# ethz-asl/laser_slam

Measured on AMD Instinct MI355X. Metric: scans_per_sec, higher is better.
Workload: dtype f32

## Files before the change

### devtools/ne_phases.py

```python
import ctypes as C, sys, os
ROOT = os.path.dirname(os.path.dirname(os.path.abspath(__file__)))
sys.path.insert(0, ROOT)
os.environ["LSGPU_SO"] = os.path.join(ROOT, "devtools", "liblsgpu_stats.so")
import numpy as np, torch
from laser_slam_amd import synth, icp
from laser_slam_amd._lib import IcpConfig, lib
n_az = int(sys.argv[1]) if len(sys.argv) > 1 else 16384
ref, rd, Tt, Ti = synth.scan_pair(n_az)
cfg = IcpConfig(); lib().lsgpu_icp_config_yaml(C.byref(cfg)); cfg.min_diff_rot, cfg.min_diff_trans = 1e-5, 1e-4
h = icp.IcpHandle(cfg)
dref, dn = h.filter_reference(torch.from_numpy(ref).cuda(), 10, 1.0, 0)
dref, dn = dref.clone(), dn.clone()
drd = torch.from_numpy(rd).cuda()
L = lib()
L.lsgpu_dev_ne_phases.argtypes = [C.c_void_p, C.POINTER(C.c_ulonglong)]
buf = (C.c_ulonglong * 24)()
h.set_reference(dref, dn); T, st = h.align(drd, Ti)
L.lsgpu_dev_ne_phases(h._h, buf); a0 = np.array(list(buf), np.float64)
h.set_reference(dref, dn); T, st = h.align(drd, Ti)
L.lsgpu_dev_ne_phases(h._h, buf); a1 = np.array(list(buf), np.float64)
d = a1 - a0
n, blocks = d[0], d[4]
print("launches %d, blocks per launch %.0f, iterations %d" % (n, blocks / n, st.iterations))
print("per block (shader cycles): prologue %.0f | main loop %.0f | wave+block reduce, hand-off %.0f" % (d[1] / blocks, d[2] / blocks, d[3] / blocks))
print("wall (us, 100 MHz clock): first start -> first loop start %.2f | first start -> last loop end %.2f | last loop end -> kernel end %.2f (update lane %.2f)"
      % (d[9] / n / 100, d[7] / n / 100, d[8] / n / 100, d[11] / n / 100))
print("tail (us): last loop end -> last block knows it is last %.2f | partials + state + set-aside loads, first sums %.2f | set-aside ranking + sums %.2f | final sums, publish %.2f" % tuple(d[16:20] / n / 100))
print("update lane (shader cycles per launch): unpack + LLT %.0f | delta, T update %.0f | trace record %.0f | checker %.0f" % tuple(d[12:16] / n))
print("distances set aside per iteration (stats build):", [t["searching"] for t in h.trace()])
```

### laser_slam_amd/csrc/lsgpu_host_math.h

```cpp
#pragma once
#include <cmath>
#include <cstring>

#if defined(__HIPCC__)
#define LSGPU_HD __host__ __device__ inline
#else
#define LSGPU_HD inline
#endif

namespace lsgpu {
namespace hostmath {

LSGPU_HD float at(const float* m, int r, int c) { return m[c * 4 + r]; }
LSGPU_HD void set(float* m, int r, int c, float v) { m[c * 4 + r] = v; }

LSGPU_HD void identity4(float* m) {
  for (int i = 0; i < 16; ++i) m[i] = (i % 5 == 0) ? 1.f : 0.f;
}

LSGPU_HD void mul4(const float* a, const float* b, float* out) {
  float t[16];
  for (int c = 0; c < 4; ++c)
    for (int r = 0; r < 4; ++r) {
      float s = at(a, r, 0) * at(b, 0, c);
// ... 158 lines not shown
    q[0] = 0.5f * t;
    t = 0.5f / t;
    q[1] = (at(T, 2, 1) - at(T, 1, 2)) * t;
    q[2] = (at(T, 0, 2) - at(T, 2, 0)) * t;
    q[3] = (at(T, 1, 0) - at(T, 0, 1)) * t;
  } else {
    int i = 0;
    if (at(T, 1, 1) > at(T, 0, 0)) i = 1;
    if (at(T, 2, 2) > at(T, i, i)) i = 2;
    const int j = (i + 1) % 3, k = (j + 1) % 3;
    t = sqrtf(at(T, i, i) - at(T, j, j) - at(T, k, k) + 1.0f);
    q[1 + i] = 0.5f * t;
    t = 0.5f / t;
    q[0] = (at(T, k, j) - at(T, j, k)) * t;
    q[1 + j] = (at(T, j, i) + at(T, i, j)) * t;
    q[1 + k] = (at(T, k, i) + at(T, i, k)) * t;
  }
}

LSGPU_HD float angular_distance(const float a[4], const float b[4]) {
  const float bw = b[0], bx = -b[1], by = -b[2], bz = -b[3];
  const float w = a[0] * bw - a[1] * bx - a[2] * by - a[3] * bz;
  const float x = a[0] * bx + a[1] * bw + a[2] * bz - a[3] * by;
  const float y = a[0] * by + a[2] * bw + a[3] * bx - a[1] * bz;
  const float z = a[0] * bz + a[3] * bw + a[1] * by - a[2] * bx;
  return 2.0f * atan2_f32(sqrtf(x * x + y * y + z * z), fabsf(w));
}

struct CheckerState {
  int counter;
  int n_hist;
};

LSGPU_HD void checker_push(CheckerState* s, float* hist, const float* T) {
  float* e = hist + 8 * s->n_hist;
  quat_from_rotation(T, e);
  e[4] = at(T, 0, 3); e[5] = at(T, 1, 3); e[6] = at(T, 2, 3);
  e[7] = s->n_hist > 0 ? fabsf(angular_distance(e, e - 8)) : 0.f;
  s->n_hist++;
}

LSGPU_HD bool checker_check(CheckerState* s, float* hist, int max_iter, int smooth, float lim_rot,
                            float lim_trans, const float* T, bool* iterate, bool* by_diff, float* out2 = nullptr) {
  if (out2) { out2[0] = 0.f; out2[1] = 0.f; }
  if (++s->counter >= max_iter) { *iterate = false; return true; }
  checker_push(s, hist, T);
  float rot = 0.f, trans = 0.f;
  const int n = s->n_hist;
  if (n > smooth) {
    for (int i = n - 1; i >= n - smooth; --i) {
      const float* a = hist + 8 * i;
      const float* b = hist + 8 * (i - 1);
      rot += a[7];
      const float dx = a[4] - b[4], dy = a[5] - b[5], dz = a[6] - b[6];
      trans += fabsf(sqrtf(dx * dx + dy * dy + dz * dz));
    }
    rot /= (float)smooth;
    trans /= (float)smooth;
    if (out2) { out2[0] = rot; out2[1] = trans; }
    if (rot < lim_rot && trans < lim_trans) { *iterate = false; *by_diff = true; }
  }
  return !(rot != rot || trans != trans);
}

}
}
```

### laser_slam_amd/csrc/lsgpu_icp.hip

```cpp
#include <cstring>
#include <cmath>
#include <cstdio>
#include <cstdlib>
#include <string>
#include <vector>
#include <chrono>
#include <functional>
#include <system_error>
#include <thread>
#include <utility>

#include <dlfcn.h>

#include <hip/hip_runtime.h>
#include <rccl/rccl.h>

#include "../../include/lsgpu_icp.h"
#include "lsgpu_grid.hip.h"
#include "lsgpu_tuning.h"
#include "lsgpu_policy.h"
#include "lsgpu_knn.hip.h"
#include "lsgpu_knn_k.hip.h"
#include "lsgpu_snf.hip.h"
#include "lsgpu_cone.hip.h"
// ... 2686 lines not shown
    pc.kmatch = kmatch; pc.chain = chain;
    pc.robust_mad = robust && ca.rb.mad; pc.robust_scale_iters = robust ? h->robust.nb_iteration_for_scale : 0;
    if (h->cone_build_in_align) { h->cone_ok = cone_wanted(h); h->cone_decided = false; }
    if (h->index_rest > 0 && (h->nr > 2 * h->index_rest_nr || 2 * h->nr < h->index_rest_nr)) h->index_rest = 0;
    const bool index_rests = h->index_rest > 0 && h->cone_ok;
    if (index_rests) { --h->index_rest; if (h->cone_build_in_align) { h->cone_build_in_align = false; h->cone_ok = false; } }
    h->pol.begin_align(h->cone_ok && !index_rests, h->cone_decided, h->cone_dense, h->cone_occupancy);
    h->pay_voxel_timed = h->pay_index_timed = false;
    if (!h->ev_pay[0]) for (auto& e : h->ev_pay) HIPC(hipEventCreate(&e));
    if (pc.lookahead && !pc.comm && !h->ev_state) HIPC(hipEventCreateWithFlags(&h->ev_state, hipEventDisableTiming));
    return LSGPU_OK;
  }

  int enqueue_iteration(const policy::Iteration& itn) {
    int r = LSGPU_OK;
    if (kmatch || chain) {
      const int np = (int)(kk * nq);
      r = run_knn_k(h, kk, Tdummy, h->state.p, itn.seed, timed);
      if (r) return r;
      ev_of_launch.push_back(h->knn_events_used ? h->knn_events_used - 1 : 0);
      r = run_select(h, h->kd2.p, np, k, false , h->state.p, true, false, 3,
                     chain ? h->cfg.trim_ratio : 0.f, chain && (ca.has_median || itn.mad));
      if (r) return r;
      if (itn.mad) { r = run_mad(h, h->kd2.p, np, h->state.p); if (r) return r; }
      ChainArgs ca_it = ca;
      ca_it.rb_recompute = itn.mad ? 1 : 0;
      lsgpu_icp::KnnEv* evk = (timed && h->knn_events_used) ? &h->knn_events[h->knn_events_used - 1] : nullptr;
      if (evk) HIPC(hipEventRecord(evk->d, h->stream));
      hipLaunchKernelGGL(ne_loop_k, dim3(nb), dim3(256), 0, h->stream, h->rdq.p, np,
                         h->state.p, h->kmatch.p, h->kd2.p, (p2p && !(robust && ca.rb.plane) && !angle) ? (const float4*)nullptr : h->nrm.p, h->hist.p, h->sel.p + 2,
                         h->counters.p + 32, h->ne_tickets.p, h->ne_partials.p, h->ne_gpartials.p, h->ne_out.p,
                         h->chk_hist.p, h->trace_dev.p, max_it, 0, (split_update && !robust && !angle) ? 0 : 1,
                         h->sel_aux.p, (uint32_t*)nullptr, 0, (uint32_t*)nullptr,
                         0, (uint32_t*)nullptr, (uint2*)nullptr, (double*)nullptr, 0, 0, ca_it);
      if (split_update && !robust && !angle)
        hipLaunchKernelGGL(update, dim3(1), dim3(64), 0, h->stream, h->state.p, h->ne_out.p,
                           h->chk_hist.p, h->trace_dev.p, max_it, 0, h->sel_aux.p);
      if (evk) HIPC(hipEventRecord(evk->e, h->stream));
      return hipGetLastError() == hipSuccess ? LSGPU_OK : LSGPU_HIP_ERROR;
    }
    if (itn.knn) {
      r = run_knn(h, Tdummy, h->state.p, itn, timed, itn.seed && itn.capped ? k : 0xFFFFFFFFu);
      if (r) return r;
      ev_of_launch.push_back(h->knn_events_used ? h->knn_events_used - 1 : 0);
    }
    if (itn.committed && h->comm) {
      RcclApi* api = rccl_api();
      comm_mark(h, true);
      if (api->GroupStart) RCCLC(api->GroupStart());
      RCCLC(api->AllReduce(h->sel_aux.p, h->sel_aux.p, kSelFailFlag, ncclUint32, ncclSum, h->comm, h->stream));
      RCCLC(api->AllReduce(h->hist.p + kHistBins, h->hist.p + kHistBins, kHistBins, ncclUint32, ncclSum, h->comm, h->stream));
      RCCLC(api->AllReduce(h->sel_win.p, h->sel_win.p, (size_t)kSelWinRows * 512, ncclUint32, ncclSum, h->comm, h->stream));
      if (api->GroupEnd) RCCLC(api->GroupEnd());
      comm_mark(h, false);
    }
    if (!itn.committed) {
      r = run_select(h, h->d2.p, (int)nq, k, false ,
                     h->state.p, true, itn.predicted, itn.full_select ? 3 : 2);
      if (r) return r;
    }
    lsgpu_icp::KnnEv* ev = (timed && itn.knn && h->knn_events_used) ? &h->knn_events[h->knn_events_used - 1] : nullptr;
    if (ev) HIPC(hipEventRecord(ev->d, h->stream));
    hipLaunchKernelGGL(ne_loop, dim3(nb), dim3(256), 0, h->stream, h->rdq.p, (int)nq,
                       h->state.p, h->prev.p, h->d2.p, p2p ? (const float4*)nullptr : h->nrm.p, h->hist.p, h->sel.p + 2,
                       h->counters.p + 32, h->ne_tickets.p, h->ne_partials.p, h->ne_gpartials.p, h->ne_out.p,
                       h->chk_hist.p, h->trace_dev.p, max_it, itn.capped ? 1 : 0, (h->comm || split_update) ? 0 : 1,
                       h->sel_aux.p, (h->comm || !tuning().fused_select) ? h->sel_win.p : nullptr, itn.committed ? 1 : 0, h->spread_cnt.p,
                       (itn.predicted && itn.knn) ? 1 : 0, h->sel_aux.p + kSelFailFlag + 2, h->amb_key.p, h->amb_val.p, tuning().sel_amb_cap,
                       (!itn.full_select && !itn.committed) ? 1 : 0, ChainArgs{});
    if (h->comm || split_update) {
      if (h->comm) comm_mark(h, true);
      if (h->comm && rccl_api()->AllReduce(h->ne_out.p, h->ne_out.p, kNe, ncclDouble, ncclSum, h->comm, h->stream) != ncclSuccess) {
        h->err = "RCCL all-reduce of the normal equations failed";
        return LSGPU_HIP_ERROR;
      }
      if (h->comm) comm_mark(h, false);
      hipLaunchKernelGGL(update, dim3(1), dim3(64), 0, h->stream, h->state.p, h->ne_out.p,
                         h->chk_hist.p, h->trace_dev.p, max_it, itn.capped ? 1 : 0, h->sel_aux.p);
    }
    if (ev) HIPC(hipEventRecord(ev->e, h->stream));
    return hipGetLastError() == hipSuccess ? LSGPU_OK : LSGPU_HIP_ERROR;
  }

  int fetch_state(int* enqueued_ahead) {
    *enqueued_ahead = 0;
    HIPC(hipMemcpyAsync(hst, h->state.p, sizeof(IcpState), hipMemcpyDeviceToHost, h->stream));
    policy::Iteration ahead_it;
    if (h->pol.lookahead_iteration(h->pol_cfg, &ahead_it)) {
      HIPC(hipEventRecord(h->ev_state, h->stream));
      const int r = enqueue_iteration(ahead_it);
      if (r) return r;
      *enqueued_ahead = 1;
      HIPC(hipEventSynchronize(h->ev_state));
      return LSGPU_OK;
    }
    return wait_stream(h);
  }

  int feed() {
    policy::Config& pc = h->pol_cfg;
    policy::State& pol = h->pol;
    int rc = enqueue_iteration(pol.plan(pc, true, pc.seed_cap && pc.cap_enabled, true, true, false));
// ... 264 lines not shown
```

### laser_slam_amd/csrc/lsgpu_solve.hip.h

```cpp
#pragma once
#include "lsgpu_common.hip.h"
#include "lsgpu_host_math.h"
#include "lsgpu_robust.h"
#include "lsgpu_normal_angle.h"
#include "../../include/lsgpu_icp.h"

namespace lsgpu {

struct SelState {
  uint32_t prefix;
  uint32_t k;
};

__device__ void find_bin(const uint32_t* __restrict__ hist, int nbins, uint32_t k, uint32_t* bin,
                         uint32_t* krem, uint32_t* sh ) {
  const int t = threadIdx.x, lane = t & 63, w = t >> 6;
  const int per = nbins / 256;
  uint32_t c[16];
  uint32_t loc = 0;
#pragma unroll
  for (int i = 0; i < 16; ++i) { c[i] = i < per ? hist[t * per + i] : 0u; loc += c[i]; }
  uint32_t incl = loc;
#pragma unroll
  for (int o = 1; o < 64; o <<= 1) {
// ... 342 lines not shown
      acc[28] += wd * ((double)res * (double)res);
      continue;
    }
    int k = 0;
#pragma unroll
    for (int a = 0; a < 6; ++a) {
#pragma unroll
      for (int c = a; c < 6; ++c) acc[k++] += (double)J[a] * (double)J[c];
    }
#pragma unroll
    for (int a = 0; a < 6; ++a) acc[21 + a] -= (double)J[a] * (double)res;
    acc[27] += 1.0;
    acc[28] += (double)res * (double)res;
  }
#pragma unroll
  for (int k = 0; k < kNe; ++k) acc[k] = ne_slot_unused<MIN>(k) ? 0.0 : wave_sum(acc[k]);
  const int w = threadIdx.x >> 6;
  if ((threadIdx.x & 63) == 0) {
#pragma unroll
    for (int k = 0; k < kNe; ++k) red[w][k] = acc[k];
  }
  __syncthreads();
  if (threadIdx.x < kNe)
    partials[(size_t)blockIdx.x * 32 + threadIdx.x] =
        ((red[0][threadIdx.x] + red[1][threadIdx.x]) + red[2][threadIdx.x]) + red[3][threadIdx.x];
}

constexpr float kCapFactor = 1.1f;

#ifdef LSGPU_KNN_STATS
__device__ unsigned long long g_ne_dbg[24] = {0, 0, 0, 0, 0, ~0ull, 0, 0, 0, 0, ~0ull, 0, 0, 0, 0, 0, 0, 0, 0, 0, 0, 0, 0, 0};
__device__ unsigned long long g_ne_tail[4];
#endif
template <int MIN, bool RB = false>
__device__ inline void icp_update_lane(IcpState* st, const double* ne_out, float* chk_hist,
                                       lsgpu_iter_trace* trace, int trace_cap, int capped_launch,
                                       uint32_t* sel_aux, int sel_failed = -1 ,
                                       const RobustIter* rb = nullptr) {
  if (st->done) return;
  if (sel_failed < 0) {
    sel_failed = (sel_aux && sel_aux[kSelFailFlag]) ? 1 : 0;
    if (sel_failed) sel_aux[kSelFailFlag] = 0u;
  }
  if (sel_failed) {
    st->sel_mode = 0;
    st->sel_fails += 1;
    st->status = kStatusSelFailed;
    st->done = 1;
    return;
  }
  const float limit = (float)ne_out[29];
  const unsigned long long nstrag = (unsigned long long)ne_out[30];
  if (capped_launch && st->cap2 < INFINITY && !(limit <= st->cap2)) {
    st->status = kStatusCapFailed;
    st->done = 1;
    return;
  }
#ifdef LSGPU_KNN_STATS
  const long long u0 = clock64();
#endif
  st->stragglers += nstrag;
  long long used = (long long)ne_out[27];
  if constexpr (RB) {
    used = rb->used;
    if (rb->mad && !(rb->scale > 0.f && rb->scale < INFINITY)) { st->status = LSGPU_NO_CONVERGENCE; st->err_code = 5; st->done = 1; return; }
    if (rb->bad > 0.0) { st->status = LSGPU_NO_CONVERGENCE; st->err_code = 6; st->done = 1; return; }
  }
  if (used <= 0) { st->status = LSGPU_NO_CONVERGENCE; st->err_code = 1; st->done = 1; return; }
  double A[36], b[6];
  float x[6], dT[16], Tn[16];
  double xd[6];
// ... 36 lines not shown
  }
  if constexpr (RB) rb->state->scale = rb->scale;
#ifdef LSGPU_KNN_STATS
  const long long u3 = clock64();
#endif
  {
    const uint32_t lb = __float_as_uint(limit), b1 = lb >> 20, b2 = (lb >> 9) & 0x7FFu;
    if (st->sel_wide) {
      const float prev = st->prev_limit;
      const bool armed = limit > 1e-30f && limit < 1e30f && prev < 1e30f && limit >= kSelArmLo * prev && limit <= kSelArmHi * prev && st->sel_fails < 2;
      const float move = armed ? fabsf(limit - prev) / prev : 1.f;
      const float f_lo = fmaxf(kSelWideLo, 1.f - 4.f * move - 0.01f), f_hi = fminf(2.f * kSelWideLo, 1.f + 4.f * move + 0.01f);
      const uint32_t lo_s = __float_as_uint(limit * f_lo) >> kSelSliceShift, hi_s = (__float_as_uint(limit * f_hi) >> kSelSliceShift) + 1u;
      st->sel_lo = lo_s << kSelSliceShift;
      st->sel_span = (hi_s - lo_s < (uint32_t)kSelSlices ? hi_s - lo_s : (uint32_t)kSelSlices) << kSelSliceShift;
      st->sel_shift = kSelSliceShift;
      st->sel_streak = armed ? st->sel_streak + 1 : 0;
      st->sel_mode = armed ? 1 : 0;
    } else {
      const uint32_t moved = b2 > st->sel_bin2 ? b2 - st->sel_bin2 : st->sel_bin2 - b2;
      st->sel_streak = (b1 == st->sel_bin1 && moved <= (uint32_t)kSelStreakBins) ? st->sel_streak + 1 : 0;
      st->sel_mode = (b1 == st->sel_bin1) ? 1 : 0;
      st->sel_lo = b1 << 20; st->sel_span = 1u << 20; st->sel_shift = 9;
    }
    st->sel_bin1 = b1;
    st->sel_bin2 = b2;
  }
  st->prev_limit = limit;
  st->cap2 = st->cap_enabled ? limit * kCapFactor : INFINITY;
  st->iter = it + 1;
  hostmath::CheckerState cs{st->counter, st->n_hist};
  bool iterate = true, by_diff = false;
  float chk2[2];
  const bool ok = hostmath::checker_check(&cs, chk_hist, st->max_iter, st->smooth, st->lim_rot,
                                          st->lim_trans, Tn, &iterate, &by_diff, chk2);
  st->chk_rot_prev = st->chk_rot; st->chk_trans_prev = st->chk_trans;
  st->chk_rot = chk2[0]; st->chk_trans = chk2[1];
  st->counter = cs.counter; st->n_hist = cs.n_hist;
#ifdef LSGPU_KNN_STATS
  {
    const long long u4 = clock64();
    g_ne_dbg[12] += (unsigned long long)(u1 - u0); g_ne_dbg[13] += (unsigned long long)(u2 - u1);
    g_ne_dbg[14] += (unsigned long long)(u3 - u2); g_ne_dbg[15] += (unsigned long long)(u4 - u3);
  }
#endif
  if (!ok) { st->status = LSGPU_NO_CONVERGENCE; st->err_code = 3; st->done = 1; return; }
  if (!iterate) { st->converged = by_diff ? 1 : 0; st->done = 1; }
}

template <int MIN>
__global__ __launch_bounds__(64) void k_icp_update(IcpState* __restrict__ st,
                                                   const double* __restrict__ ne_out,
                                                   float* __restrict__ chk_hist,
                                                   lsgpu_iter_trace* __restrict__ trace, int trace_cap,
                                                   int capped_launch, uint32_t* __restrict__ sel_aux) {
  if (threadIdx.x == 0) icp_update_lane<MIN>(st, ne_out, chk_hist, trace, trace_cap, capped_launch, sel_aux);
}


#ifndef LSGPU_NE_UNROLL
#define LSGPU_NE_UNROLL 8
#endif
constexpr int kNeUnroll = LSGPU_NE_UNROLL;
template <int MIN, int KP = 1, bool CHAIN = false, bool RB = false>
__global__ __launch_bounds__(256) void k_normal_eq_loop(const float4* __restrict__ rdq, int nq,
                                                        IcpState* __restrict__ ist,
                                                        const float4* __restrict__ match,
                                                        const float* __restrict__ d2,
                                                        const float4* __restrict__ nrm,
                                                        uint32_t* __restrict__ hist,
                                                        const SelState* __restrict__ st,
                                                        uint32_t* __restrict__ strag_count,
                                                        uint32_t* __restrict__ ticket,
                                                        double* __restrict__ partials,
                                                        double* __restrict__ gpartials,
                                                        double* __restrict__ out ,
                                                        float* __restrict__ chk_hist,
                                                        lsgpu_iter_trace* __restrict__ trace, int trace_cap,
                                                        int capped_launch, int fuse_update,
                                                        uint32_t* __restrict__ sel_aux,
                                                        uint32_t* __restrict__ hist3w ,
                                                        int committed,
                                                        uint32_t* __restrict__ spread_cnt ,
                                                        int predicted ,
                                                        uint32_t* __restrict__ amb_cnt, uint2* __restrict__ amb_key ,
                                                        double* __restrict__ amb_val ,
                                                        int amb_cap ,
                                                        int two_pass ,
                                                        ChainArgs chain ) {
  __shared__ uint32_t sc[260];
  __shared__ double fin[32];
  __shared__ double red[8][33];
  __shared__ int is_last;
  if (ist->done) return;
  const bool wide = ist->sel_wide && amb_cnt;
  const bool fused = wide && (committed || (predicted && ist->sel_mode));
  const bool plain2 = wide && !fused && two_pass;
  const bool resolve = fused || plain2;
  uint32_t s_slice = 0xFFFFFFFFu;
  uint32_t f_krem2 = 0u, f_cnt2 = 0u;
#ifdef LSGPU_KNN_STATS
  const long long c0 = clock64();
  if (threadIdx.x == 0) atomicMin(&g_ne_dbg[5], (unsigned long long)wall_clock64());
#endif
  Mat34 T;
#pragma unroll
  for (int i = 0; i < 12; ++i) T.m[i] = ist->T_rows[i];
  float limit;
  bool sel_ok = true;
  if (fused) {
    __shared__ uint32_t wsum[4], fres[4];
    const int t = threadIdx.x, lane = t & 63, w = t >> 6;
    const uint4* h4 = reinterpret_cast<const uint4*>(hist + kHistBins) + t * (kSelSlices / 256 / 4);
    static_assert(kSelSlices == 256 * 16, "16 slices per thread");
    uint4 c4[4];
#pragma unroll
    for (int i = 0; i < 4; ++i) c4[i] = h4[i];
    uint32_t bel = t < kSelBelowSlots ? sel_aux[t * kSelBelowStride] : 0u;
    const uint32_t k = st[-2].k;
    uint32_t c[16];
#pragma unroll
    for (int i = 0; i < 4; ++i) { c[4 * i] = c4[i].x; c[4 * i + 1] = c4[i].y; c[4 * i + 2] = c4[i].z; c[4 * i + 3] = c4[i].w; }
    uint32_t loc = 0u;
#pragma unroll
    for (int i = 0; i < 16; ++i) loc += c[i];
    uint32_t incl = loc;
#pragma unroll
// ... 74 lines not shown
    if constexpr (RB) { if (!chain.has_trim) limit = INFINITY; }
    if constexpr (CHAIN) {
      if (chain.has_median) limit = fminf(limit, chain.med_factor * select_limit(chain.hist_med + 2 * kHistBins, chain.sel_med + 2, sc));
      limit = fminf(limit, chain.max2);
    }
    if (wide) {
      const uint32_t lb = __float_as_uint(limit), sl = lb >> kSelSliceShift;
      const uint32_t i0 = (sl << (kSelSliceShift - 9)) & (uint32_t)(kHistBins - 1);
      uint32_t cnt = 0u;
      for (uint32_t i = 0; i < (1u << (kSelSliceShift - 9)); ++i) cnt += hist[kHistBins + i0 + i];
      if (cnt <= (uint32_t)amb_cap) { s_slice = sl; f_cnt2 = cnt; }
    }
  }
#ifdef LSGPU_KNN_STATS
  const long long c1 = clock64();
  if (threadIdx.x == 0) atomicMin(&g_ne_dbg[10], (unsigned long long)wall_clock64());
#endif
  float rb_scale = 1.f, rb_med = 0.f;
  double rb_cnt = 0.0, rb_bad = 0.0;
  if constexpr (RB) {
    if (chain.rb.mad) {
      rb_med = chain.rb_state->median;
      if (chain.rb_recompute) rb_scale = sqrtf(select_limit(chain.rb_hist + 2 * kHistBins, chain.rb_sel + 2, sc));
      else rb_scale = chain.rb_state->scale;
    }
  }
  const bool rb_normals = MIN != kPointToPoint || (RB && chain.rb.plane);
  const float* na_rn = nullptr;
  if constexpr (CHAIN) na_rn = chain.na_rn;
  double na_rej = 0.0;
  double acc[kNe];
#pragma unroll
  for (int k = 0; k < kNe; ++k) acc[k] = 0.0;
  const int stride = gridDim.x * 256;
  for (int j0 = blockIdx.x * 256 + threadIdx.x; j0 < (sel_ok ? nq : 0); j0 += kNeUnroll * stride) {
    float dd[kNeUnroll]; float4 qq[kNeUnroll], rr[kNeUnroll], nn[kNeUnroll]; bool use[kNeUnroll], amb[kNeUnroll];
#pragma unroll
    for (int u = 0; u < kNeUnroll; ++u) {
      const int j = j0 + u * stride;
      use[u] = j < nq;
      dd[u] = use[u] ? d2[j] : INFINITY;
      {
        const uint32_t sl = __float_as_uint(dd[u]) >> kSelSliceShift;
        const bool in_s = sl == s_slice;
        bool inl = resolve ? sl <= s_slice : dd[u] <= limit;
        if constexpr (CHAIN) inl = inl && chain.lo2 <= dd[u];
        amb[u] = use[u] && inl && in_s;
        use[u] = use[u] && inl;
      }
      qq[u] = use[u] ? match[j] : make_float4(0.f, 0.f, 0.f, __int_as_float(-1));
      if constexpr (KP > 1) rr[u] = use[u] ? rdq[j / KP] : make_float4(0.f, 0.f, 0.f, 0.f);
      else rr[u] = use[u] ? rdq[j] : make_float4(0.f, 0.f, 0.f, 0.f);
      use[u] = use[u] && __float_as_int(qq[u].w) >= 0;
    }
#pragma unroll
    for (int u = 0; u < kNeUnroll; ++u) {
      if constexpr (MIN != kPointToPoint) nn[u] = use[u] ? nrm[__float_as_int(qq[u].w)] : make_float4(0.f, 0.f, 0.f, 0.f);
      else if constexpr (RB) nn[u] = (use[u] && (rb_normals || na_rn)) ? nrm[__float_as_int(qq[u].w)] : make_float4(0.f, 0.f, 0.f, 0.f);
      else if constexpr (CHAIN) nn[u] = (use[u] && na_rn) ? nrm[__float_as_int(qq[u].w)] : make_float4(0.f, 0.f, 0.f, 0.f);
    }
#pragma unroll
    for (int u = 0; u < kNeUnroll; ++u) {
    if (!use[u]) continue;
    const float4 q = qq[u];
    const float4 r = rr[u];
    if constexpr (CHAIN) {
      if (na_rn) {
        const float* rn = na_rn + 3 * (size_t)__float_as_uint(r.w);
        if (!normal_angle::keep(T.m, rn[0], rn[1], rn[2], nn[u].x, nn[u].y, nn[u].z, chain.na_eps)) { na_rej += 1.0; continue; }
      }
    }
    const float3 p = xform(T, r.x, r.y, r.z);
    if constexpr (MIN == kPointToPoint) {
      double v[16];
// ... 58 lines not shown
                           __ATOMIC_RELAXED, __HIP_MEMORY_SCOPE_AGENT);
      }
      continue;
    }
    if constexpr (RB) {
      const float wf = robust::weight(chain.rb.fct, chain.rb.plane ? res * res : dd[u], rb_scale, chain.rb.k, chain.rb.approx2);
      if (!(fabsf(wf) < INFINITY)) { rb_bad += 1.0; continue; }
      if (!(wf > 0.f)) continue;
      rb_cnt += 1.0;
      const double wd = (double)wf;
      int k = 0;
#pragma unroll
      for (int a = 0; a < 6; ++a) {
#pragma unroll
        for (int c = a; c < 6; ++c) acc[k++] += wd * ((double)J[a] * (double)J[c]);
      }
#pragma unroll
      for (int a = 0; a < 6; ++a) acc[21 + a] -= wd * ((double)J[a] * (double)res);
      acc[27] += wd;
      acc[28] += wd * ((double)res * (double)res);
      continue;
    }
    int k = 0;
#pragma unroll
    for (int a = 0; a < 6; ++a) {
#pragma unroll
      for (int c = a; c < 6; ++c) acc[k++] += (double)J[a] * (double)J[c];
    }
#pragma unroll
    for (int a = 0; a < 6; ++a) acc[21 + a] -= (double)J[a] * (double)res;
    acc[27] += 1.0;
    acc[28] += (double)res * (double)res;
    }
  }
#ifdef LSGPU_KNN_STATS
  asm volatile("s_waitcnt vmcnt(0)" ::: "memory");
  const long long c2 = clock64();
  if (threadIdx.x == 0) atomicMax(&g_ne_dbg[6], (unsigned long long)wall_clock64());
#endif
#pragma unroll
  for (int k = 0; k < kNe; ++k) acc[k] = ne_slot_unused<MIN>(k) ? 0.0 : wave_sum(acc[k]);
  const int w = threadIdx.x >> 6;
  if constexpr (RB) { rb_cnt = wave_sum(rb_cnt); rb_bad = wave_sum(rb_bad); }
  if constexpr (CHAIN) { if (na_rn) na_rej = wave_sum(na_rej); }
  if ((threadIdx.x & 63) == 0) {
#pragma unroll
    for (int k = 0; k < kNe; ++k) red[w][k] = acc[k];
    if constexpr (RB) { red[w][29] = rb_cnt; red[w][30] = rb_bad; }
    if constexpr (CHAIN) red[w][31] = na_rej;
  }
  __syncthreads();
  if (threadIdx.x < (RB ? kNe + 2 : kNe) || (CHAIN && threadIdx.x == 31))
    __hip_atomic_store(&partials[(size_t)blockIdx.x * 32 + threadIdx.x],
                       ((red[0][threadIdx.x] + red[1][threadIdx.x]) + red[2][threadIdx.x]) + red[3][threadIdx.x],
                       __ATOMIC_RELAXED, __HIP_MEMORY_SCOPE_AGENT);
#if (defined(__gfx950__) || defined(__gfx942__)) && !defined(LSGPU_NE_FENCED)
  asm volatile("s_waitcnt vmcnt(0)" ::: "memory");
#else
  __builtin_amdgcn_fence(__ATOMIC_RELEASE, "agent");
  asm volatile("s_waitcnt vmcnt(0)" ::: "memory");
#endif
  __syncthreads();
  if (threadIdx.x == 0) {
    const uint32_t t = __hip_atomic_fetch_add(ticket, 1u, __ATOMIC_RELAXED, __HIP_MEMORY_SCOPE_AGENT);
    is_last = (t == gridDim.x - 1);
#ifdef LSGPU_KNN_STATS
    const long long c3 = clock64();
    atomicAdd(&g_ne_dbg[1], (unsigned long long)(c1 - c0)); atomicAdd(&g_ne_dbg[2], (unsigned long long)(c2 - c1));
    atomicAdd(&g_ne_dbg[3], (unsigned long long)(c3 - c2)); atomicAdd(&g_ne_dbg[4], 1ull);
#endif
  }
  __syncthreads();
  if (!is_last) return;
#ifdef LSGPU_KNN_STATS
  if (threadIdx.x == 0) g_ne_tail[0] = (unsigned long long)wall_clock64();
#endif
#if !((defined(__gfx950__) || defined(__gfx942__)) && !defined(LSGPU_NE_FENCED))
  __builtin_amdgcn_fence(__ATOMIC_ACQUIRE, "agent");
#endif
  __shared__ IcpState st_sh;
  __shared__ uint32_t fail_sh, cnt_sh[2];
  constexpr int kStWords = (int)(sizeof(IcpState) / sizeof(uint32_t));
  uint32_t* sw = reinterpret_cast<uint32_t*>(&st_sh);
  uint32_t* gw = reinterpret_cast<uint32_t*>(ist);
  uint32_t st_word[(kStWords + 255) / 256];
  if (fuse_update) {
#pragma unroll
    for (int i = 0; i < (kStWords + 255) / 256; ++i)
      st_word[i] = (int)threadIdx.x + 256 * i < kStWords ? gw[threadIdx.x + 256 * i] : 0u;
  }
  const bool s_on = sel_ok && s_slice != 0xFFFFFFFFu;
  __shared__ __attribute__((aligned(16))) uint32_t akj[kSelAmbCap];
  __shared__ __attribute__((aligned(16))) uint32_t akb[kSelAmbCap];
  __shared__ uint32_t aord[kSelAmbCap];
  __shared__ uint32_t alim_sh, am_sh;
  __shared__ double red2[8][33];
  constexpr int kAmbLds = 64;
  __shared__ double aval[kAmbLds * 32];
  uint32_t an = 0u;
  unsigned long long akey = 0ull;
  double av[kAmbLds * 32 / 256];
  if (s_on) {
    an = __hip_atomic_load(amb_cnt, __ATOMIC_RELAXED, __HIP_MEMORY_SCOPE_AGENT);
    const uint32_t kmax = f_cnt2 ? f_cnt2 - 1u : 0u, vmax = kmax * 32u + 31u;
    akey = __hip_atomic_load(reinterpret_cast<unsigned long long*>(&amb_key[threadIdx.x < kmax ? threadIdx.x : kmax]), __ATOMIC_RELAXED, __HIP_MEMORY_SCOPE_AGENT);
#pragma unroll
    for (int u = 0; u < kAmbLds * 32 / 256; ++u) {
      const uint32_t i = threadIdx.x + 256u * (uint32_t)u;
      av[u] = __hip_atomic_load(&amb_val[i < vmax ? i : vmax], __ATOMIC_RELAXED, __HIP_MEMORY_SCOPE_AGENT);
    }
  }
  uint32_t fail_word = 0u, ns_word = 0u, nw_word = 0u;
  if (threadIdx.x == 255) {
    if (sel_aux) fail_word = sel_aux[kSelFailFlag];
    ns_word = __hip_atomic_load(strag_count, __ATOMIC_RELAXED, __HIP_MEMORY_SCOPE_AGENT);
    nw_word = __hip_atomic_load(strag_count + 2, __ATOMIC_RELAXED, __HIP_MEMORY_SCOPE_AGENT);
  }
  {
    const int col = threadIdx.x & 31, slice = threadIdx.x >> 5;
    const uint32_t per = (gridDim.x + 7u) / 8u;
    const uint32_t r0 = (uint32_t)slice * per, r1 = r0 + per < gridDim.x ? r0 + per : gridDim.x;
    double t = 0.0;
    uint32_t r = r0;
    for (; r + 16 <= r1; r += 16) {
      double v[16];
#pragma unroll
      for (int u = 0; u < 16; ++u)
        v[u] = __hip_atomic_load(&partials[(size_t)(r + u) * 32 + col], __ATOMIC_RELAXED, __HIP_MEMORY_SCOPE_AGENT);
#pragma unroll
      for (int u = 0; u < 16; ++u) t += v[u];
    }
    for (; r < r1; ++r)
      t += __hip_atomic_load(&partials[(size_t)r * 32 + col], __ATOMIC_RELAXED, __HIP_MEMORY_SCOPE_AGENT);
    red[slice][col] = t;
  }
  if (fuse_update) {
#pragma unroll
    for (int i = 0; i < (kStWords + 255) / 256; ++i)
      if ((int)threadIdx.x + 256 * i < kStWords) sw[threadIdx.x + 256 * i] = st_word[i];
  }
  if (s_on) {
#pragma unroll
    for (int u = 0; u < kAmbLds * 32 / 256; ++u) aval[threadIdx.x + 256 * u] = av[u];
    const uint32_t n_in = an < (uint32_t)kSelAmbCap ? an : (uint32_t)kSelAmbCap;
    akj[threadIdx.x] = threadIdx.x < n_in ? (uint32_t)akey : 0xFFFFFFFFu;
    akb[threadIdx.x] = threadIdx.x < n_in ? (uint32_t)(akey >> 32) : 0xFFFFFFFFu;
    if (threadIdx.x == 0) { alim_sh = resolve ? 0xFFFFFFFFu : __float_as_uint(limit); am_sh = 0u; }
  }
  __syncthreads();
#ifdef LSGPU_KNN_STATS
  if (threadIdx.x == 0) g_ne_tail[1] = (unsigned long long)wall_clock64();
#endif
  bool amb_ok = true;
  if (s_on) {
    if (resolve) amb_ok = an == f_cnt2;
    const uint32_t n = amb_ok ? (an < (uint32_t)kSelAmbCap ? an : (uint32_t)kSelAmbCap) : 0u;
    const uint32_t mb = akb[threadIdx.x], mj = akj[threadIdx.x];
    if (resolve) {
      if (threadIdx.x < n) {
        uint32_t cl = 0u, cle = 0u;
        for (uint32_t e0 = 0; e0 < n; e0 += 8u) {
          const uint4 b0 = *reinterpret_cast<const uint4*>(&akb[e0]), b1 = *reinterpret_cast<const uint4*>(&akb[e0 + 4u]);
          const uint32_t eb[8] = {b0.x, b0.y, b0.z, b0.w, b1.x, b1.y, b1.z, b1.w};
#pragma unroll
          for (int q = 0; q < 8; ++q) { cl += eb[q] < mb ? 1u : 0u; cle += eb[q] <= mb ? 1u : 0u; }
        }
        if (cl <= f_krem2 && f_krem2 < cle) alim_sh = mb;
      }
      __syncthreads();
    }
    const uint32_t lim_bits = alim_sh;
    amb_ok = amb_ok && lim_bits != 0xFFFFFFFFu;
    limit = __uint_as_float(lim_bits);
// ... 66 lines not shown
#ifdef LSGPU_KNN_STATS
    const double nw_dbg = s_on ? (double)an : nw;
    out[31] = nw_dbg; fin[31] = nw_dbg;
#else
    out[31] = nw; fin[31] = nw;
#endif
    __hip_atomic_store(strag_count, 0u, __ATOMIC_RELAXED, __HIP_MEMORY_SCOPE_AGENT);
    __hip_atomic_store(strag_count + 2, 0u, __ATOMIC_RELAXED, __HIP_MEMORY_SCOPE_AGENT);
    __hip_atomic_store(ticket, 0u, __ATOMIC_RELAXED, __HIP_MEMORY_SCOPE_AGENT);
    if (spread_cnt) {
      const uint32_t n = __hip_atomic_load(spread_cnt + 1, __ATOMIC_RELAXED, __HIP_MEMORY_SCOPE_AGENT);
      const uint32_t nc = n < (uint32_t)kFrontMax ? n : (uint32_t)kFrontMax;
      __hip_atomic_store(spread_cnt, nc, __ATOMIC_RELAXED, __HIP_MEMORY_SCOPE_AGENT);
      if (fuse_update) st_sh.n_spread = nc; else ist->n_spread = nc;
    }
  }
#ifdef LSGPU_KNN_STATS
  unsigned long long w_pre = 0;
  if (threadIdx.x == 0) w_pre = (unsigned long long)wall_clock64();
#endif
  __syncthreads();
  if (threadIdx.x == 0) {
    if constexpr (CHAIN) {
      if (na_rn && chain.na_trace && !st_sh.done && st_sh.iter < trace_cap) {
        lsgpu_normal_angle_trace& nt = chain.na_trace[st_sh.iter];
        nt.rejected = (long long)red[2][32]; nt.eps = chain.na_eps; nt.reserved = 0;
      }
    }
    if constexpr (RB) {
      RobustIter ri;
      ri.used = (long long)red[0][32]; ri.bad = red[1][32]; ri.scale = rb_scale; ri.median = rb_med;
      ri.recomputed = (chain.rb.mad && chain.rb_recompute) ? 1 : 0; ri.mad = chain.rb.mad;
      ri.state = chain.rb_state; ri.trace = chain.rb_trace;
      icp_update_lane<MIN, true>(&st_sh, fin, chk_hist, trace, trace_cap, capped_launch, nullptr, (int)fail_sh, &ri);
    } else if (fuse_update) icp_update_lane<MIN>(&st_sh, fin, chk_hist, trace, trace_cap, capped_launch, nullptr, (int)fail_sh);
    else if (sel_aux && fail_sh) sel_aux[kSelFailFlag] = 1u;
  } else if (threadIdx.x >= 64) {
    const int t = (int)threadIdx.x - 64;
    for (int i = t; i < 3 * kHistBins; i += 192) hist[i] = 0u;
    if (sel_aux && t < kSelBelowSlots) sel_aux[t * kSelBelowStride] = 0u;
    if (sel_aux && fuse_update && t == kSelBelowSlots) sel_aux[kSelFailFlag] = 0u;
    if (hist3w) {
      uint4* w4 = reinterpret_cast<uint4*>(hist3w);
      for (int i = t; i < kSelWinRows * 512 / 4; i += 192) w4[i] = make_uint4(0u, 0u, 0u, 0u);
    }
  }
  if (fuse_update) {
    __syncthreads();
#pragma unroll
    for (int i = 0; i < (kStWords + 255) / 256; ++i)
      if ((int)threadIdx.x + 256 * i < kStWords) gw[threadIdx.x + 256 * i] = sw[threadIdx.x + 256 * i];
  }
#ifdef LSGPU_KNN_STATS
  if (threadIdx.x == 0) {
    const unsigned long long wend = (unsigned long long)wall_clock64();
    const unsigned long long w0 = g_ne_dbg[5], w2 = g_ne_dbg[6], w1 = g_ne_dbg[10];
    g_ne_dbg[0] += 1ull; g_ne_dbg[7] += w2 - w0; g_ne_dbg[8] += wend - w2; g_ne_dbg[9] += w1 - w0;
    g_ne_dbg[11] += wend - w_pre;
    g_ne_dbg[16] += g_ne_tail[0] - w2; g_ne_dbg[17] += g_ne_tail[1] - g_ne_tail[0]; g_ne_dbg[18] += g_ne_tail[2] - g_ne_tail[1]; g_ne_dbg[19] += w_pre - g_ne_tail[2];
    g_ne_dbg[5] = ~0ull; g_ne_dbg[6] = 0ull; g_ne_dbg[10] = ~0ull;
  }
#endif
}

__global__ __launch_bounds__(1024) void k_ne_final(const double* __restrict__ partials, int nblocks,
                                                   double* __restrict__ out) {
  __shared__ double sh[32][33];
  const int col = threadIdx.x & 31, grp = threadIdx.x >> 5;
  double s = 0.0;
  if (col < kNe)
    for (int b = grp; b < nblocks; b += 32) s += partials[(size_t)b * 32 + col];
  sh[grp][col] = s;
  __syncthreads();
  if (threadIdx.x < kNe) {
    double t = 0.0;
    for (int r = 0; r < 32; ++r) t += sh[r][threadIdx.x];
    out[threadIdx.x] = t;
  }
}

}
```

### laser_slam_amd/csrc/lsgpu_tuning.h

```cpp

#pragma once
#include <cstdio>
#include <cstdlib>
#include <cstring>

extern char** environ;

namespace lsgpu {

struct Tuning {
  int query_order = -1;
  float q_elev = 0.f, q_sect = 0.f;
  float gap = 0.002f;
  int chunk_budget = 512, chunk_budget_wide = 1024;
  int wide_iters = 3;
  float route_r = 0.02f;
  int route_chunks = 1024;
  int route_heavy_max = 1024;
  int route_dense = 512;
  bool predict_select = true, commit_select = true, comm_commit = true, seed_cap = true;
  int sel_amb_cap = 256;
  bool two_pass_select = true;
  bool short_last_group = true;
  bool fused_select = true;
  bool lazy_need = true;
  bool lane_split = true;
  bool lookahead = true;
  bool index_rest = true;
  bool side_stream = true;
  int front_guess = 2048;
  int sort_items = 0;
  bool ssn_sort_levels = false;
  int ssn_root = 0;
  int ne_blocks = 256;
  bool split_update = false;
  double comm_timeout_ms = 30000.0;
  int knn_dbg = 0;
  bool cone = true;
  bool cone_probe = true;
  int cone_rows = 128, cone_cols = 8192, cone_from = 2;
  float cone_max_occupancy = 7.0f;
  float cone_heavy_steps = 1024.f;
  float cone_heavy_share = 0.07f;
};

namespace tuning_detail {
inline bool flag(const char* name) { return getenv(name) != nullptr; }
inline double number(const char* name, double def, double lo, double hi) {
  const char* e = getenv(name);
  if (!e) return def;
  char* end = nullptr;
  const double v = strtod(e, &end);
  if (end == e || *end != '\0' || !(v >= lo && v <= hi)) {
    fprintf(stderr, "liblsgpu_icp: %s=%s is not a number in [%g, %g]; using the default %g\n", name, e, lo, hi, def);
    return def;
  }
  return v;
}
inline Tuning read() {
  Tuning t;
  t.query_order = (int)number("LSGPU_QUERY_ORDER", -1, -1, 1);
  t.q_elev = (float)number("LSGPU_Q_ELEV", 0, 0, 45);
  t.q_sect = (float)number("LSGPU_Q_SECT", 0, 0, 45);
  t.gap = (float)number("LSGPU_GAP", 0.002, 0, 1);
  t.chunk_budget = (int)number("LSGPU_BUDGET", 512, 1, 1 << 20);
  t.chunk_budget_wide = (int)number("LSGPU_BUDGET_WIDE", 1024, 1, 1 << 20);
  t.wide_iters = (int)number("LSGPU_WIDE_ITERS", 3, 0, 1 << 20);
  t.route_r = (float)number("LSGPU_ROUTE_R", 0.02, 1e-6, 1e6);
  t.route_chunks = (int)number("LSGPU_ROUTE_CHUNKS", 1024, 1, 1 << 30);
  t.route_heavy_max = (int)number("LSGPU_ROUTE_HEAVY_MAX", 1024, -1, 1 << 30);
  t.route_dense = (int)number("LSGPU_ROUTE_DENSE", 512, 1, 1 << 30);
  t.split_update = flag("LSGPU_SPLIT_UPDATE");
  t.predict_select = !flag("LSGPU_NO_PREDICT") && !t.split_update;
  t.commit_select = !flag("LSGPU_NO_COMMIT");
  t.fused_select = !flag("LSGPU_NO_FUSED_SELECT");
  t.short_last_group = !flag("LSGPU_FULL_GROUPS");
  t.two_pass_select = !flag("LSGPU_THREE_PASS_SELECT");
  t.sel_amb_cap = (int)number("LSGPU_SEL_AMB_CAP", 256, 0, 256);
  t.comm_commit = !flag("LSGPU_NO_COMM_COMMIT");
  t.seed_cap = !flag("LSGPU_NO_SEED_CAP");
  t.lazy_need = !flag("LSGPU_NO_LAZY");
  t.lane_split = !flag("LSGPU_NO_SPLIT");
  t.side_stream = !flag("LSGPU_NO_SIDE_STREAM");
  t.lookahead = !flag("LSGPU_NO_LOOKAHEAD");
  t.index_rest = !flag("LSGPU_NO_INDEX_REST");
  t.front_guess = (int)number("LSGPU_FRONT_GUESS", 2048, 0, 8192);
  t.sort_items = (int)number("LSGPU_SORT_ITEMS", 0, 0, 16);
  if (t.sort_items != 0 && t.sort_items != 4 && t.sort_items != 8 && t.sort_items != 16) {
    fprintf(stderr, "liblsgpu_icp: LSGPU_SORT_ITEMS must be 4, 8 or 16; choosing by size\n");
    t.sort_items = 0;
  }
  t.ssn_sort_levels = flag("LSGPU_SSN_SORT_LEVELS");
  t.ssn_root = (int)number("LSGPU_SSN_ROOT", 0, 0, 8192);
  if (t.ssn_root != 0 && t.ssn_root != 2048 && t.ssn_root != 4096 && t.ssn_root != 8192) {
    fprintf(stderr, "liblsgpu_icp: LSGPU_SSN_ROOT must be 2048, 4096 or 8192; choosing by size\n");
    t.ssn_root = 0;
  }
  t.ne_blocks = (int)number("LSGPU_NE_BLOCKS", 256, 64, 2048);
  t.comm_timeout_ms = number("LSGPU_COMM_TIMEOUT_MS", 30000, 1, 1e9);
  t.knn_dbg = (int)number("LSGPU_KNN_DBG", 0, 0, 1 << 20);
  t.cone = !flag("LSGPU_NO_CONE");
  t.cone_probe = !flag("LSGPU_NO_CONE_PROBE");
  t.cone_from = (int)number("LSGPU_CONE_FROM", 2, 1, 1 << 20);
  t.cone_max_occupancy = (float)number("LSGPU_CONE_MAX_OCC", 7.0, 0.0, 1e9);
  t.cone_heavy_steps = (float)number("LSGPU_CONE_HEAVY_STEPS", 1024.0, 0.0, 1e9);
  t.cone_heavy_share = (float)number("LSGPU_CONE_HEAVY_SHARE", 0.07, 0.0, 2.0);
  t.cone_rows = (int)number("LSGPU_CONE_ROWS", 128, 8, 1024);
  t.cone_cols = (int)number("LSGPU_CONE_COLS", 8192, 64, 65536) & ~3;
  static const char* known[] = {"LSGPU_QUERY_ORDER", "LSGPU_Q_ELEV", "LSGPU_Q_SECT", "LSGPU_GAP", "LSGPU_BUDGET", "LSGPU_BUDGET_WIDE", "LSGPU_WIDE_ITERS",
                                "LSGPU_ROUTE_R", "LSGPU_ROUTE_CHUNKS", "LSGPU_ROUTE_HEAVY_MAX", "LSGPU_ROUTE_DENSE", "LSGPU_SPLIT_UPDATE", "LSGPU_NO_PREDICT", "LSGPU_NO_COMMIT",
                                "LSGPU_NO_COMM_COMMIT", "LSGPU_NO_SEED_CAP", "LSGPU_NO_LAZY", "LSGPU_NO_SPLIT", "LSGPU_NO_SIDE_STREAM", "LSGPU_NO_LOOKAHEAD", "LSGPU_NO_INDEX_REST", "LSGPU_CELLS_SPLIT", "LSGPU_NO_FUSED_SELECT", "LSGPU_FULL_GROUPS", "LSGPU_THREE_PASS_SELECT", "LSGPU_SEL_AMB_CAP", "LSGPU_FRONT_GUESS",
                                "LSGPU_SORT_ITEMS", "LSGPU_SSN_ROOT", "LSGPU_SSN_SORT_LEVELS",
                                "LSGPU_NE_BLOCKS", "LSGPU_COMM_TIMEOUT_MS", "LSGPU_KNN_DBG", "LSGPU_NO_CONE", "LSGPU_NO_CONE_PROBE", "LSGPU_CONE_ROWS", "LSGPU_CONE_COLS", "LSGPU_CONE_FROM", "LSGPU_CONE_MAX_OCC", "LSGPU_CONE_HEAVY_STEPS", "LSGPU_CONE_HEAVY_SHARE",
                                "LSGPU_SO", "LSGPU_STATS_SO", "LSGPU_BATCH_POOLS", "LSGPU_BATCH_UNIQ", "LSGPU_GS_DEBUG", "LSGPU_GOLDEN_DIR", "LSGPU_SEQ_PERTURB", "LSGPU_SEQ_POSES", "LSGPU_TEST_INPUT_FILTERS",
                                nullptr};
  for (char** e = environ; e && *e; ++e) {
    if (strncmp(*e, "LSGPU_", 6) != 0) continue;
    const char* eq = strchr(*e, '=');
    const size_t len = eq ? (size_t)(eq - *e) : strlen(*e);
    bool ok = false;
    for (const char** k = known; *k; ++k) ok = ok || (strlen(*k) == len && strncmp(*k, *e, len) == 0);
    if (!ok) fprintf(stderr, "liblsgpu_icp: unknown switch %.*s ignored (see csrc/lsgpu_tuning.h)\n", (int)len, *e);
  }
  return t;
}
}

inline const Tuning& tuning() {
  static const Tuning t = tuning_detail::read();
  return t;
}

}
```

Measured before the change: 250.3.

## Shorten normal-equation kernel tail with prefetch, LDS checker window, batched partial loads

Three latency-hiding changes go into the fused normal-equation/update kernel. The first distance loads are issued before the prologue so their latency overlaps setup. The convergence checker's recent history window is staged into shared memory during the reduction tail, and the new entry is written back afterwards, which takes global loads off the serial update lane. Partial sums are read in batches of 32 to keep more loads in flight. Each change has an env switch to turn it off, and together they add register pressure and shared memory.

```diff
diff --git a/devtools/ne_phases.py b/devtools/ne_phases.py
--- a/devtools/ne_phases.py
+++ b/devtools/ne_phases.py
@@ -1,7 +1,7 @@
 import ctypes as C, sys, os
 ROOT = os.path.dirname(os.path.dirname(os.path.abspath(__file__)))
 sys.path.insert(0, ROOT)
-os.environ["LSGPU_SO"] = os.path.join(ROOT, "devtools", "liblsgpu_stats.so")
+os.environ.setdefault("LSGPU_SO", os.path.join(ROOT, "devtools", "liblsgpu_stats.so"))
 import numpy as np, torch
 from laser_slam_amd import synth, icp
 from laser_slam_amd._lib import IcpConfig, lib
diff --git a/laser_slam_amd/csrc/lsgpu_host_math.h b/laser_slam_amd/csrc/lsgpu_host_math.h
--- a/laser_slam_amd/csrc/lsgpu_host_math.h
+++ b/laser_slam_amd/csrc/lsgpu_host_math.h
@@ -214,8 +214,8 @@
   int n_hist;
 };
 
-LSGPU_HD void checker_push(CheckerState* s, float* hist, const float* T) {
-  float* e = hist + 8 * s->n_hist;
+LSGPU_HD void checker_push(CheckerState* s, float* hist, const float* T, int off = 0) {
+  float* e = hist + 8 * (s->n_hist - off);
   quat_from_rotation(T, e);
   e[4] = at(T, 0, 3); e[5] = at(T, 1, 3); e[6] = at(T, 2, 3);
   e[7] = s->n_hist > 0 ? fabsf(angular_distance(e, e - 8)) : 0.f;
@@ -223,16 +223,17 @@
 }
 
 LSGPU_HD bool checker_check(CheckerState* s, float* hist, int max_iter, int smooth, float lim_rot,
-                            float lim_trans, const float* T, bool* iterate, bool* by_diff, float* out2 = nullptr) {
+                            float lim_trans, const float* T, bool* iterate, bool* by_diff, float* out2 = nullptr,
+                            int off = 0) {
   if (out2) { out2[0] = 0.f; out2[1] = 0.f; }
   if (++s->counter >= max_iter) { *iterate = false; return true; }
-  checker_push(s, hist, T);
+  checker_push(s, hist, T, off);
   float rot = 0.f, trans = 0.f;
   const int n = s->n_hist;
   if (n > smooth) {
     for (int i = n - 1; i >= n - smooth; --i) {
-      const float* a = hist + 8 * i;
-      const float* b = hist + 8 * (i - 1);
+      const float* a = hist + 8 * (i - off);
+      const float* b = hist + 8 * (i - 1 - off);
       rot += a[7];
       const float dx = a[4] - b[4], dy = a[5] - b[5], dz = a[6] - b[6];
       trans += fabsf(sqrtf(dx * dx + dy * dy + dz * dz));
diff --git a/laser_slam_amd/csrc/lsgpu_icp.hip b/laser_slam_amd/csrc/lsgpu_icp.hip
--- a/laser_slam_amd/csrc/lsgpu_icp.hip
+++ b/laser_slam_amd/csrc/lsgpu_icp.hip
@@ -2742,7 +2742,7 @@
                          h->counters.p + 32, h->ne_tickets.p, h->ne_partials.p, h->ne_gpartials.p, h->ne_out.p,
                          h->chk_hist.p, h->trace_dev.p, max_it, 0, (split_update && !robust && !angle) ? 0 : 1,
                          h->sel_aux.p, (uint32_t*)nullptr, 0, (uint32_t*)nullptr,
-                         0, (uint32_t*)nullptr, (uint2*)nullptr, (double*)nullptr, 0, 0, ca_it);
+                         0, (uint32_t*)nullptr, (uint2*)nullptr, (double*)nullptr, 0, 0, tuning().ne_plain_tail, ca_it);
       if (split_update && !robust && !angle)
         hipLaunchKernelGGL(update, dim3(1), dim3(64), 0, h->stream, h->state.p, h->ne_out.p,
                            h->chk_hist.p, h->trace_dev.p, max_it, 0, h->sel_aux.p);
@@ -2777,7 +2777,7 @@
                        h->chk_hist.p, h->trace_dev.p, max_it, itn.capped ? 1 : 0, (h->comm || split_update) ? 0 : 1,
                        h->sel_aux.p, (h->comm || !tuning().fused_select) ? h->sel_win.p : nullptr, itn.committed ? 1 : 0, h->spread_cnt.p,
                        (itn.predicted && itn.knn) ? 1 : 0, h->sel_aux.p + kSelFailFlag + 2, h->amb_key.p, h->amb_val.p, tuning().sel_amb_cap,
-                       (!itn.full_select && !itn.committed) ? 1 : 0, ChainArgs{});
+                       (!itn.full_select && !itn.committed) ? 1 : 0, tuning().ne_plain_tail, ChainArgs{});
     if (h->comm || split_update) {
       if (h->comm) comm_mark(h, true);
       if (h->comm && rccl_api()->AllReduce(h->ne_out.p, h->ne_out.p, kNe, ncclDouble, ncclSum, h->comm, h->stream) != ncclSuccess) {
diff --git a/laser_slam_amd/csrc/lsgpu_solve.hip.h b/laser_slam_amd/csrc/lsgpu_solve.hip.h
--- a/laser_slam_amd/csrc/lsgpu_solve.hip.h
+++ b/laser_slam_amd/csrc/lsgpu_solve.hip.h
@@ -398,11 +398,14 @@
 __device__ unsigned long long g_ne_dbg[24] = {0, 0, 0, 0, 0, ~0ull, 0, 0, 0, 0, ~0ull, 0, 0, 0, 0, 0, 0, 0, 0, 0, 0, 0, 0, 0};
 __device__ unsigned long long g_ne_tail[4];
 #endif
+constexpr int kChkWin = 8;
+constexpr int kNePlainChk = 2, kNePlainBatch = 4, kNePlainLoads = 8;
 template <int MIN, bool RB = false>
 __device__ inline void icp_update_lane(IcpState* st, const double* ne_out, float* chk_hist,
                                        lsgpu_iter_trace* trace, int trace_cap, int capped_launch,
                                        uint32_t* sel_aux, int sel_failed = -1 ,
-                                       const RobustIter* rb = nullptr) {
+                                       const RobustIter* rb = nullptr, float* chk_win = nullptr ,
+                                       bool chk_lds = false) {
   if (st->done) return;
   if (sel_failed < 0) {
     sel_failed = (sel_aux && sel_aux[kSelFailFlag]) ? 1 : 0;
@@ -505,8 +508,12 @@
   hostmath::CheckerState cs{st->counter, st->n_hist};
   bool iterate = true, by_diff = false;
   float chk2[2];
-  const bool ok = hostmath::checker_check(&cs, chk_hist, st->max_iter, st->smooth, st->lim_rot,
-                                          st->lim_trans, Tn, &iterate, &by_diff, chk2);
+  bool ok;
+  if (chk_lds && st->smooth < kChkWin)
+    ok = hostmath::checker_check(&cs, chk_win, st->max_iter, st->smooth, st->lim_rot, st->lim_trans, Tn, &iterate, &by_diff, chk2,
+                                 cs.n_hist - (kChkWin - 1));
+  else
+    ok = hostmath::checker_check(&cs, chk_hist, st->max_iter, st->smooth, st->lim_rot, st->lim_trans, Tn, &iterate, &by_diff, chk2);
   st->chk_rot_prev = st->chk_rot; st->chk_trans_prev = st->chk_trans;
   st->chk_rot = chk2[0]; st->chk_trans = chk2[1];
   st->counter = cs.counter; st->n_hist = cs.n_hist;
@@ -560,12 +567,21 @@
                                                         double* __restrict__ amb_val ,
                                                         int amb_cap ,
                                                         int two_pass ,
+                                                        int plain_tail ,
                                                         ChainArgs chain ) {
   __shared__ uint32_t sc[260];
   __shared__ double fin[32];
   __shared__ double red[8][33];
   __shared__ int is_last;
   if (ist->done) return;
+  const int n_hist0 = ist->n_hist;
+  const int stride = gridDim.x * 256;
+  float dpre[kNeUnroll];
+#pragma unroll
+  for (int u = 0; u < kNeUnroll; ++u) {
+    const int j = blockIdx.x * 256 + threadIdx.x + u * stride;
+    dpre[u] = (!(plain_tail & kNePlainLoads) && j < nq) ? d2[j] : INFINITY;
+  }
   const bool wide = ist->sel_wide && amb_cnt;
   const bool fused = wide && (committed || (predicted && ist->sel_mode));
   const bool plain2 = wide && !fused && two_pass;
@@ -706,14 +722,14 @@
   double acc[kNe];
 #pragma unroll
   for (int k = 0; k < kNe; ++k) acc[k] = 0.0;
-  const int stride = gridDim.x * 256;
+  bool first = !(plain_tail & kNePlainLoads);
   for (int j0 = blockIdx.x * 256 + threadIdx.x; j0 < (sel_ok ? nq : 0); j0 += kNeUnroll * stride) {
     float dd[kNeUnroll]; float4 qq[kNeUnroll], rr[kNeUnroll], nn[kNeUnroll]; bool use[kNeUnroll], amb[kNeUnroll];
 #pragma unroll
     for (int u = 0; u < kNeUnroll; ++u) {
       const int j = j0 + u * stride;
       use[u] = j < nq;
-      dd[u] = use[u] ? d2[j] : INFINITY;
+      dd[u] = first ? dpre[u] : (use[u] ? d2[j] : INFINITY);
       {
         const uint32_t sl = __float_as_uint(dd[u]) >> kSelSliceShift;
         const bool in_s = sl == s_slice;
@@ -838,6 +854,7 @@
     acc[27] += 1.0;
     acc[28] += (double)res * (double)res;
     }
+    first = false;
   }
 #ifdef LSGPU_KNN_STATS
   asm volatile("s_waitcnt vmcnt(0)" ::: "memory");
@@ -895,6 +912,12 @@
     for (int i = 0; i < (kStWords + 255) / 256; ++i)
       st_word[i] = (int)threadIdx.x + 256 * i < kStWords ? gw[threadIdx.x + 256 * i] : 0u;
   }
+  const bool lds_chk = fuse_update && !(plain_tail & kNePlainChk);
+  __shared__ float chk_sh[8 * kChkWin];
+  const int chk_i = 8 * (n_hist0 - (kChkWin - 1)) + ((int)threadIdx.x - 64);
+  const bool chk_mine = lds_chk && threadIdx.x >= 64 && threadIdx.x < 64 + 8 * (kChkWin - 1);
+  float chk_word = 0.f;
+  if (chk_mine && chk_i >= 0) chk_word = chk_hist[chk_i];
   const bool s_on = sel_ok && s_slice != 0xFFFFFFFFu;
   __shared__ __attribute__((aligned(16))) uint32_t akj[kSelAmbCap];
   __shared__ __attribute__((aligned(16))) uint32_t akb[kSelAmbCap];
@@ -928,6 +951,16 @@
     const uint32_t r0 = (uint32_t)slice * per, r1 = r0 + per < gridDim.x ? r0 + per : gridDim.x;
     double t = 0.0;
     uint32_t r = r0;
+    if (!(plain_tail & kNePlainBatch)) {
+      for (; r + 32 <= r1; r += 32) {
+        double v[32];
+#pragma unroll
+        for (int u = 0; u < 32; ++u)
+          v[u] = __hip_atomic_load(&partials[(size_t)(r + u) * 32 + col], __ATOMIC_RELAXED, __HIP_MEMORY_SCOPE_AGENT);
+#pragma unroll
+        for (int u = 0; u < 32; ++u) t += v[u];
+      }
+    }
     for (; r + 16 <= r1; r += 16) {
       double v[16];
 #pragma unroll
@@ -945,6 +978,7 @@
     for (int i = 0; i < (kStWords + 255) / 256; ++i)
       if ((int)threadIdx.x + 256 * i < kStWords) sw[threadIdx.x + 256 * i] = st_word[i];
   }
+  if (chk_mine) chk_sh[threadIdx.x - 64] = chk_word;
   if (s_on) {
 #pragma unroll
     for (int u = 0; u < kAmbLds * 32 / 256; ++u) aval[threadIdx.x + 256 * u] = av[u];
@@ -1077,8 +1111,8 @@
       ri.used = (long long)red[0][32]; ri.bad = red[1][32]; ri.scale = rb_scale; ri.median = rb_med;
       ri.recomputed = (chain.rb.mad && chain.rb_recompute) ? 1 : 0; ri.mad = chain.rb.mad;
       ri.state = chain.rb_state; ri.trace = chain.rb_trace;
-      icp_update_lane<MIN, true>(&st_sh, fin, chk_hist, trace, trace_cap, capped_launch, nullptr, (int)fail_sh, &ri);
-    } else if (fuse_update) icp_update_lane<MIN>(&st_sh, fin, chk_hist, trace, trace_cap, capped_launch, nullptr, (int)fail_sh);
+      icp_update_lane<MIN, true>(&st_sh, fin, chk_hist, trace, trace_cap, capped_launch, nullptr, (int)fail_sh, &ri, chk_sh, lds_chk);
+    } else if (fuse_update) icp_update_lane<MIN>(&st_sh, fin, chk_hist, trace, trace_cap, capped_launch, nullptr, (int)fail_sh, nullptr, chk_sh, lds_chk);
     else if (sel_aux && fail_sh) sel_aux[kSelFailFlag] = 1u;
   } else if (threadIdx.x >= 64) {
     const int t = (int)threadIdx.x - 64;
@@ -1095,6 +1129,9 @@
 #pragma unroll
     for (int i = 0; i < (kStWords + 255) / 256; ++i)
       if ((int)threadIdx.x + 256 * i < kStWords) gw[threadIdx.x + 256 * i] = sw[threadIdx.x + 256 * i];
+    const int t2 = (int)threadIdx.x - 64;
+    if (lds_chk && t2 >= 0 && t2 < 8 && st_sh.smooth < kChkWin && st_sh.n_hist == n_hist0 + 1)
+      chk_hist[8 * n_hist0 + t2] = chk_sh[8 * (kChkWin - 1) + t2];
   }
 #ifdef LSGPU_KNN_STATS
   if (threadIdx.x == 0) {
diff --git a/laser_slam_amd/csrc/lsgpu_tuning.h b/laser_slam_amd/csrc/lsgpu_tuning.h
--- a/laser_slam_amd/csrc/lsgpu_tuning.h
+++ b/laser_slam_amd/csrc/lsgpu_tuning.h
@@ -33,6 +33,7 @@
   bool ssn_sort_levels = false;
   int ssn_root = 0;
   int ne_blocks = 256;
+  int ne_plain_tail = 0;
   bool split_update = false;
   double comm_timeout_ms = 30000.0;
   int knn_dbg = 0;
@@ -71,6 +72,8 @@
   t.route_heavy_max = (int)number("LSGPU_ROUTE_HEAVY_MAX", 1024, -1, 1 << 30);
   t.route_dense = (int)number("LSGPU_ROUTE_DENSE", 512, 1, 1 << 30);
   t.split_update = flag("LSGPU_SPLIT_UPDATE");
+  t.ne_plain_tail = (int)number("LSGPU_NE_PLAIN_TAIL", 0, 0, 15);
+  t.ne_plain_tail = (t.ne_plain_tail & 1) ? 14 : t.ne_plain_tail;
   t.predict_select = !flag("LSGPU_NO_PREDICT") && !t.split_update;
   t.commit_select = !flag("LSGPU_NO_COMMIT");
   t.fused_select = !flag("LSGPU_NO_FUSED_SELECT");
@@ -111,7 +114,7 @@
                                 "LSGPU_ROUTE_R", "LSGPU_ROUTE_CHUNKS", "LSGPU_ROUTE_HEAVY_MAX", "LSGPU_ROUTE_DENSE", "LSGPU_SPLIT_UPDATE", "LSGPU_NO_PREDICT", "LSGPU_NO_COMMIT",
                                 "LSGPU_NO_COMM_COMMIT", "LSGPU_NO_SEED_CAP", "LSGPU_NO_LAZY", "LSGPU_NO_SPLIT", "LSGPU_NO_SIDE_STREAM", "LSGPU_NO_LOOKAHEAD", "LSGPU_NO_INDEX_REST", "LSGPU_CELLS_SPLIT", "LSGPU_NO_FUSED_SELECT", "LSGPU_FULL_GROUPS", "LSGPU_THREE_PASS_SELECT", "LSGPU_SEL_AMB_CAP", "LSGPU_FRONT_GUESS",
                                 "LSGPU_SORT_ITEMS", "LSGPU_SSN_ROOT", "LSGPU_SSN_SORT_LEVELS",
-                                "LSGPU_NE_BLOCKS", "LSGPU_COMM_TIMEOUT_MS", "LSGPU_KNN_DBG", "LSGPU_NO_CONE", "LSGPU_NO_CONE_PROBE", "LSGPU_CONE_ROWS", "LSGPU_CONE_COLS", "LSGPU_CONE_FROM", "LSGPU_CONE_MAX_OCC", "LSGPU_CONE_HEAVY_STEPS", "LSGPU_CONE_HEAVY_SHARE",
+                                "LSGPU_NE_BLOCKS", "LSGPU_NE_PLAIN_TAIL", "LSGPU_COMM_TIMEOUT_MS", "LSGPU_KNN_DBG", "LSGPU_NO_CONE", "LSGPU_NO_CONE_PROBE", "LSGPU_CONE_ROWS", "LSGPU_CONE_COLS", "LSGPU_CONE_FROM", "LSGPU_CONE_MAX_OCC", "LSGPU_CONE_HEAVY_STEPS", "LSGPU_CONE_HEAVY_SHARE",
                                 "LSGPU_SO", "LSGPU_STATS_SO", "LSGPU_BATCH_POOLS", "LSGPU_BATCH_UNIQ", "LSGPU_GS_DEBUG", "LSGPU_GOLDEN_DIR", "LSGPU_SEQ_PERTURB", "LSGPU_SEQ_POSES", "LSGPU_TEST_INPUT_FILTERS",
                                 nullptr};
   for (char** e = environ; e && *e; ++e) {
```

Result: no change. 251.3 (median of 6 runs) (+0.4%).
